# shrubb/latent-pose-reenactment

Measured on AMD Instinct MI355X. Metric: train-step images/sec at 256x256 bs=8, higher is better.
Workload: dtype mixed 16-bit MFMA operands, fp32 accumulate, fp32 activations / weights / optimizer state; 1 GPU; default.yaml meta-training step (configs[2]): ResNeXt50 identity encoder over 8 frames + MobileNetV2 pose encoder (both trained, forward + backward on hand-written gfx950 kernels), G, D with the 98000x512 label embedding, VGG19/VGGFace/featmat/adversarial/dis_embed/dice criterions, Adam, EMA; image_size=256, per_gpu_batch=8, global_batch=8, parallelism=dp1, precision_mode=default assignment (LP_PREC=f16), padding=zero, launch_mode=hipgraph

## Files before the change

### latent_pose_reenactment_amd/build.py

```python
import os
import subprocess
import sys
import time
from concurrent.futures import ThreadPoolExecutor

HERE = os.path.dirname(os.path.abspath(__file__))
CSRC = os.path.join(HERE, 'csrc')
INCLUDE = os.path.join(os.path.dirname(HERE), 'include')
LIB = os.path.join(HERE, 'liblp_hip.so')
SOURCES = ['lp_api.hip', 'elementwise.hip', 'norm_bwd.hip', 'tanh_head.hip', 'spectral_norm.hip', 'act_pack.hip', 'conv_dma.hip', 'conv_pipe.hip', 'conv_wgrad.hip', 'conv_thin.hip', 'conv_stem8.hip', 'linear_crop.hip', 'mobilenet.hip', 'resnext.hip', 'reflect_border.hip', 'stickman.hip']
FLAGS = ['--offload-arch=gfx950', '-O3', '-std=c++17', '-fPIC', '-I', INCLUDE, '-I', CSRC]


def _newer(a, b):
    return not os.path.exists(b) or os.path.getmtime(a) > os.path.getmtime(b)


def build(force: bool = False, verbose: bool = True) -> str:
    hipcc = os.environ.get('HIPCC', '/opt/rocm/bin/hipcc')
    objdir = os.path.join(HERE, 'build')
    os.makedirs(objdir, exist_ok=True)
    headers = [os.path.join(CSRC, f) for f in os.listdir(CSRC) if f.endswith('.h')] + [os.path.join(INCLUDE, 'lp_hip.h')]
    jobs = []
    for src in SOURCES:
        s = os.path.join(CSRC, src)
        o = os.path.join(objdir, src.replace('.hip', '.o'))
        if force or _newer(s, o) or any(_newer(h, o) for h in headers):
            jobs.append((s, o))

    def compile_one(job):
        s, o = job
        t_start = time.time()
        cmd = [hipcc] + FLAGS + ['-c', s, '-o', o]
        if verbose:
            print('[lp build]', ' '.join(cmd), flush=True)
        r = subprocess.run(cmd, capture_output=True, text=True)
        if r.returncode != 0:
            raise RuntimeError(f'hipcc failed for {s}:\n{r.stderr}')
        os.utime(o, (t_start, t_start))
        return o

    with ThreadPoolExecutor(max_workers=4) as ex:
        list(ex.map(compile_one, jobs))
    objs = [os.path.join(objdir, s.replace('.hip', '.o')) for s in SOURCES]
    if jobs or not os.path.exists(LIB):
        cmd = [hipcc, '--offload-arch=gfx950', '-shared', '-fPIC', '-o', LIB] + objs
        if verbose:
            print('[lp build]', ' '.join(cmd), flush=True)
        r = subprocess.run(cmd, capture_output=True, text=True)
        if r.returncode != 0:
            raise RuntimeError(f'link failed:\n{r.stderr}')
    return LIB


if __name__ == '__main__':
    print(build(force='--force' in sys.argv))
```

### latent_pose_reenactment_amd/csrc/conv_common.h

```cpp
#pragma once
#include "lp_common.h"
#include <stdlib.h>

struct Conv16Params {
    const uint16_t* a_hi; const uint16_t* a_lo; const uint16_t* w_hi; const uint16_t* w_lo;
    float* y;
    const float* bias; const float* res; const float* alpha; const float* alpha2;
    const uint16_t* mask16;
    uint16_t* o_hi; uint16_t* o_lo;
    int o_relu;
    float* amax;
    float* part; long long part_bytes;
    int N, H, W, Hin, Win, Cin, C8, Cout, Co8, CinP, CoutP;
    int res_shift;
    int lTH, lTW, lNB, tiles_x, tiles_y;
    int hit;
    int a_dbuf;
    int ksplit;
    float* stats;
    long long stats_cap;
    int stats_rows;
    int xcd_map, ntiles, nco;
    int phase;
    int grouped;
};

static inline int ilog2_floor(int v) { int l = 0; while ((1 << (l + 1)) <= v) ++l; return l; }

__device__ __forceinline__ bool conv16_block(const Conv16Params& p, int& tile, int& cob) {
    if (!p.xcd_map) { tile = (int)blockIdx.x; cob = (int)blockIdx.y; return true; }
    const int id = (int)blockIdx.x, x = id & 7, j = id >> 3;
    if (p.xcd_map == 2) { tile = id % p.ntiles; cob = id / p.ntiles; return cob < p.nco; }
    const int per = (p.ntiles + 7) >> 3;
    cob = j % p.nco;
    const int k = j / p.nco;
    tile = x * per + k;
    return k < per && tile < p.ntiles;
}

static inline dim3 conv16_grid(Conv16Params& p, int ntiles, int nco, int gz = 1) {
    static const int on = getenv("LP_CONV_XCD") ? atoi(getenv("LP_CONV_XCD")) : 1;
    p.ntiles = ntiles; p.nco = nco;
    p.xcd_map = (on && nco > 1 && ntiles >= 16) ? on : 0;
    if (!p.xcd_map) return dim3(ntiles, nco, gz);
    return dim3(((ntiles + 7) / 8) * 8 * nco, 1, gz);
}

static inline void choose_tile(int BM, int N, int H, int W, int* lTH, int* lTW, int* lNB) {
    int lbm = ilog2_floor(BM);
    int ltw = ilog2_floor(W); if (ltw > 4) ltw = 4;
    int lth = ilog2_floor(H); if (lth > lbm - ltw) lth = lbm - ltw;
    if (lth < 1) lth = 1;
    if (ltw < 1) ltw = 1;
    int lnb = lbm - ltw - lth; if (lnb < 0) lnb = 0;
    while (lnb > 0 && (1 << (lnb - 1)) >= N) --lnb;
    *lTH = lth; *lTW = ltw; *lNB = lnb;
}

int lp_conv_pipe_launch(Conv16Params& p, int ups, int prec, hipStream_t s);
int lp_conv1x1_pipe_launch(Conv16Params& p, int prec, hipStream_t s);

template <int WM, int WN, int MR, int NR, int PREC, int MRP>
__device__ __forceinline__ void conv16_epilogue(const Conv16Params& p, f32x4_t (&acc)[MR][NR], unsigned char* smem, int wave_d, int wm, int wn,
                                                int lane, int n0, int y0, int x0, int co0, int NBv, int tile_index, int ph = -1) {
    constexpr bool SPLIT = (PREC == LP_PREC_BF16X3), F16 = (PREC == LP_PREC_F16);
    float alpha = p.alpha ? *p.alpha : 1.f;
    if (p.alpha2) alpha *= *p.alpha2;
    if ((p.Cout & 3) == 0) {
        constexpr int WR = MR * 16, WC = NR * 16, LDW = WC + 4;
        __syncthreads();
        float* tile = (float*)smem + wave_d * (MRP * 16 * LDW);
        constexpr int C4 = WC / 4;
        constexpr int RPP = 64 / C4;
        const int c4 = lane % C4, rsub = lane / C4;
        const int co = co0 + wn * WC + c4 * 4;
        float4 bv = make_float4(0.f, 0.f, 0.f, 0.f);
        if (p.bias && co < p.Cout) bv = *(const float4*)(p.bias + co);
        float am = 0.f;
        float st_n = 0.f, st_ref[4] = {0.f, 0.f, 0.f, 0.f}, st_d[4] = {0.f, 0.f, 0.f, 0.f}, st_q[4] = {0.f, 0.f, 0.f, 0.f};
#pragma unroll
        for (int mp = 0; mp < MR; mp += MRP) {
#pragma unroll
            for (int mr = mp; mr < mp + MRP; ++mr)
#pragma unroll
                for (int nr = 0; nr < NR; ++nr)
#pragma unroll
                    for (int r = 0; r < 4; ++r)
                        tile[((mr - mp) * 16 + (lane >> 4) * 4 + r) * LDW + nr * 16 + (lane & 15)] = acc[mr][nr][r];
#pragma unroll 4
        for (int r0 = mp * 16; r0 < (mp + MRP) * 16; r0 += RPP) {
            const int row = r0 + rsub;
            const int m = wm * WR + row;
            int nb, py, px;
            tile_row_linear(m, p.lTH, p.lTW, nb, py, px);
            const int n = n0 + nb;
            int oyy = y0 + py, oxx = x0 + px;
            bool inside = nb < NBv && n < p.N && co < p.Cout;
            if (ph >= 0) { inside = inside && oyy < p.Hin && oxx < p.Win; oyy = 2 * oyy + (ph >> 1); oxx = 2 * oxx + (ph & 1); }
            else inside = inside && oyy < p.H && oxx < p.W;
            if (inside) {
                float4 v = *(const float4*)(tile + (row - mp * 16) * LDW + c4 * 4);
                if (p.ksplit > 1) {
                    const size_t pixs = (size_t)(n * p.H + oyy) * p.W + oxx;
                    *(float4*)(p.part + ((size_t)blockIdx.z * p.N * p.H * p.W + pixs) * p.Cout + co) = v;
                    continue;
                }
                v.x = fmaf(v.x, alpha, bv.x); v.y = fmaf(v.y, alpha, bv.y); v.z = fmaf(v.z, alpha, bv.z); v.w = fmaf(v.w, alpha, bv.w);
                if (p.res) {
                    const float4 rv = *(const float4*)(p.res + ((size_t)(n * (p.H >> p.res_shift) + (oyy >> p.res_shift)) * (p.W >> p.res_shift)
                                                                + (oxx >> p.res_shift)) * p.Cout + co);
                    v.x += rv.x; v.y += rv.y; v.z += rv.z; v.w += rv.w;
                }
                const size_t pix = (size_t)(n * p.H + oyy) * p.W + oxx;
                if (p.mask16) {
                    const ushort4 mv = *(const ushort4*)(p.mask16 + pix * p.Co8 + co);
                    v.x = (mv.x - 1u) < 0x7fffu ? v.x : 0.f; v.y = (mv.y - 1u) < 0x7fffu ? v.y : 0.f;
                    v.z = (mv.z - 1u) < 0x7fffu ? v.z : 0.f; v.w = (mv.w - 1u) < 0x7fffu ? v.w : 0.f;
                }
                if (p.o_relu & 2) { v.x = fmaxf(v.x, 0.f); v.y = fmaxf(v.y, 0.f); v.z = fmaxf(v.z, 0.f); v.w = fmaxf(v.w, 0.f); }
                if (p.y) *(float4*)(p.y + pix * p.Cout + co) = v;
                am = lp_amax4(am, v);
                if (p.stats) {
                    const float o4[4] = {v.x, v.y, v.z, v.w};
                    if (st_n == 0.f) { st_ref[0] = v.x; st_ref[1] = v.y; st_ref[2] = v.z; st_ref[3] = v.w; }
#pragma unroll
                    for (int j = 0; j < 4; ++j) { const float d = o4[j] - st_ref[j]; st_d[j] += d; st_q[j] = fmaf(d, d, st_q[j]); }
                    st_n += 1.f;
                }
                if (p.o_hi) {
                    float o[4] = {v.x, v.y, v.z, v.w};
                    ushort4 oh, ol;
                    uint16_t* ohp = (uint16_t*)&oh; uint16_t* olp = (uint16_t*)&ol;
#pragma unroll
                    for (int j = 0; j < 4; ++j) {
                        const float q = (p.o_relu & 1) ? fmaxf(o[j], 0.f) : o[j];
                        ohp[j] = lp_f32_to_op16<F16>(q);
                        if (SPLIT) olp[j] = lp_f32_to_op16<false>(q - lp_op16_to_f32<false>(ohp[j]));
                    }
                    *(ushort4*)(p.o_hi + pix * p.Co8 + co) = oh;
                    if (SPLIT) *(ushort4*)(p.o_lo + pix * p.Co8 + co) = ol;
                }
            }
        }
        }
        if (p.amax && p.ksplit == 1) lp_amax_commit(am, p.amax, blockIdx.x + blockIdx.y * 7u);
        if (p.stats && p.ksplit == 1) {
            float mean[4], m2[4];
#pragma unroll
            for (int j = 0; j < 4; ++j) {
                mean[j] = 0.f; m2[j] = 0.f;
                if (st_n > 0.f) { mean[j] = st_ref[j] + st_d[j] / st_n; m2[j] = fmaxf(st_q[j] - st_d[j] * st_d[j] / st_n, 0.f); }
            }
#pragma unroll
            for (int o = C4; o < 64; o <<= 1) {
                const float nb_ = __shfl_xor(st_n, o, 64);
                float mb[4], qb[4];
#pragma unroll
                for (int j = 0; j < 4; ++j) { mb[j] = __shfl_xor(mean[j], o, 64); qb[j] = __shfl_xor(m2[j], o, 64); }
                const float nn = st_n + nb_;
                if (nn > 0.f) {
                    const float fb = nb_ / nn, fab = st_n * fb;
#pragma unroll
                    for (int j = 0; j < 4; ++j) { const float d = mb[j] - mean[j]; mean[j] = fmaf(d, fb, mean[j]); m2[j] += qb[j] + d * d * fab; }
                }
                st_n = nn;
            }
            if (rsub == 0 && co < p.Cout) {
                float* o = p.stats + ((size_t)(tile_index * WM + wm) * p.Cout + co) * 3;
#pragma unroll
                for (int j = 0; j < 4; ++j) { o[j * 3 + 0] = st_n; o[j * 3 + 1] = mean[j]; o[j * 3 + 2] = m2[j]; }
            }
        }
        return;
    }
    float am_s = 0.f;
#pragma unroll
    for (int mr = 0; mr < MR; ++mr) {
#pragma unroll
        for (int r = 0; r < 4; ++r) {
            const int m = wm * (MR * 16) + mr * 16 + (lane >> 4) * 4 + r;
            int nb, py, px;
            tile_row_linear(m, p.lTH, p.lTW, nb, py, px);
            const int n = n0 + nb, oyy = y0 + py, oxx = x0 + px;
            if (nb >= NBv || n >= p.N || oyy >= p.H || oxx >= p.W) continue;
            const size_t pixi = (size_t)(n * p.H + oyy) * p.W + oxx;
            const size_t pix = pixi * p.Cout;
            size_t rpix = 0;
            if (p.res) rpix = ((size_t)(n * (p.H >> p.res_shift) + (oyy >> p.res_shift)) * (p.W >> p.res_shift) + (oxx >> p.res_shift)) * p.Cout;
#pragma unroll
            for (int nr = 0; nr < NR; ++nr) {
                const int co = co0 + wn * (NR * 16) + nr * 16 + (lane & 15);
                if (co < p.Cout) {
                    float v = acc[mr][nr][r] * alpha;
                    if (p.bias) v += p.bias[co];
                    if (p.res) v += p.res[rpix + co];
                    if (p.mask16 && !((unsigned)(p.mask16[pixi * p.Co8 + co] - 1u) < 0x7fffu)) v = 0.f;
                    if (p.y) p.y[pix + co] = v;
                    am_s = fmaxf(am_s, fabsf(v));
                    if (p.o_hi) {
                        const float q = (p.o_relu & 1) ? fmaxf(v, 0.f) : v;
                        const uint16_t h = lp_f32_to_op16<F16>(q);
                        p.o_hi[pixi * p.Co8 + co] = h;
                        if (SPLIT) p.o_lo[pixi * p.Co8 + co] = lp_f32_to_op16<false>(q - lp_op16_to_f32<false>(h));
                    }
                }
            }
        }
    }
    if (p.amax) lp_amax_commit(am_s, p.amax, blockIdx.x + blockIdx.y * 7u);
}
```

### latent_pose_reenactment_amd/csrc/conv_dma.hip

```cpp
#include "lp_common.h"
#include "conv_common.h"
#include "lp_hip.h"
#include "lp_internal.h"
#include <stdlib.h>
#include <type_traits>

__device__ __attribute__((aligned(64))) unsigned int lp_zero_page[16];


template <int KS, bool UPS, int WM, int WN, int MR, int NR, int PREC, bool PP, int NBUF = 2, int CC = 32, bool GH = false>
#ifndef LP_PP_MINW
#define LP_PP_MINW 2
#endif
#ifndef LP_X3_1X1_MINW
#define LP_X3_1X1_MINW 3
#endif
__global__ __launch_bounds__(WM * WN * 64 * (PP ? 2 : 1), (PP && PREC != LP_PREC_BF16X3) ? LP_PP_MINW : (!PP && NBUF == 2 && WM * WN == 4 && PREC != LP_PREC_BF16X3) ? 2 :
                             (KS == 1 && !PP && WM * WN == 4 && PREC == LP_PREC_BF16X3) ? LP_X3_1X1_MINW : 1)
void conv_dma_kernel(Conv16Params p) {
    constexpr int ROWB = CC * 2;
    constexpr int SL = CC / 8, RPI = 64 / SL;
    constexpr int KK = CC / 32;
    static_assert(CC == 32 || CC == 64, "32- or 64-channel chunks");
    constexpr bool SPLIT = (PREC == LP_PREC_BF16X3), F16 = (PREC == LP_PREC_F16);
// ... 276 lines not shown
        float4 v = *(const float4*)(p.part + i * 4);
        for (int z = 1; z < p.ksplit; ++z) {
            const float4 q = *(const float4*)(p.part + z * slice + i * 4);
            v.x += q.x; v.y += q.y; v.z += q.z; v.w += q.w;
        }
        float4 bv = make_float4(0.f, 0.f, 0.f, 0.f);
        if (p.bias) bv = *(const float4*)(p.bias + co);
        v.x = fmaf(v.x, alpha, bv.x); v.y = fmaf(v.y, alpha, bv.y); v.z = fmaf(v.z, alpha, bv.z); v.w = fmaf(v.w, alpha, bv.w);
        if (p.res) {
            const int ox = (int)(pix % p.W); const size_t t = pix / p.W;
            const int oy = (int)(t % p.H), n = (int)(t / p.H);
            const float4 rv = *(const float4*)(p.res + ((size_t)(n * (p.H >> p.res_shift) + (oy >> p.res_shift)) * (p.W >> p.res_shift)
                                                        + (ox >> p.res_shift)) * p.Cout + co);
            v.x += rv.x; v.y += rv.y; v.z += rv.z; v.w += rv.w;
        }
        if (p.mask16) {
            const ushort4 mv = *(const ushort4*)(p.mask16 + pix * p.Co8 + co);
            v.x = (mv.x - 1u) < 0x7fffu ? v.x : 0.f; v.y = (mv.y - 1u) < 0x7fffu ? v.y : 0.f;
            v.z = (mv.z - 1u) < 0x7fffu ? v.z : 0.f; v.w = (mv.w - 1u) < 0x7fffu ? v.w : 0.f;
        }
        if (p.o_relu & 2) { v.x = fmaxf(v.x, 0.f); v.y = fmaxf(v.y, 0.f); v.z = fmaxf(v.z, 0.f); v.w = fmaxf(v.w, 0.f); }
        if (p.y) *(float4*)(p.y + pix * p.Cout + co) = v;
        am = lp_amax4(am, v);
        if (p.o_hi) {
            float o[4] = {v.x, v.y, v.z, v.w};
            ushort4 oh, ol;
            uint16_t* ohp = (uint16_t*)&oh; uint16_t* olp = (uint16_t*)&ol;
#pragma unroll
            for (int j = 0; j < 4; ++j) {
                const float q = (p.o_relu & 1) ? fmaxf(o[j], 0.f) : o[j];
                ohp[j] = lp_f32_to_op16<F16>(q);
                if (SPLIT) olp[j] = lp_f32_to_op16<false>(q - lp_op16_to_f32<false>(ohp[j]));
            }
            *(ushort4*)(p.o_hi + pix * p.Co8 + co) = oh;
            if (SPLIT) *(ushort4*)(p.o_lo + pix * p.Co8 + co) = ol;
        }
    }
    if (p.amax) lp_amax_commit(am, p.amax, blockIdx.x);
}

template <int KS, bool UPS, int WM, int WN, int MR, int NR, int PREC, bool PP, int NBUF = 2, int CC = 32, bool GH = false>
static int launch_v(Conv16Params& p, size_t lds, dim3 grid, hipStream_t stream) {
    auto kern = conv_dma_kernel<KS, UPS, WM, WN, MR, NR, PREC, PP, NBUF, CC, GH>;
    static thread_local int attr_dev = -1;
    int dev = 0;
    if (hipGetDevice(&dev) != hipSuccess) return lp_set_error(LP_ERR_HIP, "hipGetDevice failed");
    if (attr_dev != dev) {
        if (hipFuncSetAttribute((const void*)kern, hipFuncAttributeMaxDynamicSharedMemorySize, 160 * 1024) != hipSuccess)
            return lp_set_error(LP_ERR_HIP, "hipFuncSetAttribute failed");
        attr_dev = dev;
    }
    hipLaunchKernelGGL(kern, grid, dim3(WM * WN * 64 * (PP ? 2 : 1)), lds, stream, p);
    return lp_check_launch("conv_dma");
}

template <int KS, bool UPS, int WM, int WN, int MR, int NR, int PREC, int CC = 32, bool GH = false>
static int launch_conv16(Conv16Params& p, hipStream_t stream) {
    constexpr int BM = WM * MR * 16, BN = WN * NR * 16, NWAVE = WM * WN;
    constexpr bool SPLIT = (PREC == LP_PREC_BF16X3);
    constexpr int ROWB = CC * 2, RPI = 64 / (CC / 8);
    constexpr size_t B_BUF = (size_t)KS * BN * ROWB * (SPLIT ? 2 : 1);
    constexpr size_t LDS_MAX = 160 * 1024;
    constexpr int AIT = ((BM == 128) ? (NWAVE == 8 ? 3 : 5) : 6) * (CC / 32) - (CC == 64 ? 1 : 0);
    if (p.CinP % CC) return lp_set_error(LP_ERR_ARG, "conv16: padded input channels must be a multiple of the chunk size");
    const bool phf = (KS == 2) && p.phase == 1, phd = (KS == 2) && p.phase == 2;
    const int GHt = phf ? p.Hin : p.H, GWt = phf ? p.Win : p.W;
    choose_tile(BM, p.N, GHt, GWt, &p.lTH, &p.lTW, &p.lNB);
    int HH, HW, halo_px;
    for (;;) {
        const int TH = 1 << p.lTH, TW = 1 << p.lTW, NBv = 1 << p.lNB;
        if (KS == 1) { HH = TH; HW = TW; } else if (KS == 2) { HH = TH + 1; HW = TW + 1; } else if (UPS) { HH = TH / 2 + 2; HW = TW / 2 + 2; } else { HH = TH + 2; HW = TW + 2; }
        halo_px = NBv * HH * HW;
        if ((halo_px + RPI - 1) / RPI <= AIT * NWAVE || p.lNB == 0) break;
        --p.lNB;
    }
    const int TH = 1 << p.lTH, TW = 1 << p.lTW, NBv = 1 << p.lNB;
    p.tiles_x = (GWt + TW - 1) / TW; p.tiles_y = (GHt + TH - 1) / TH;
    const int NH = (halo_px + RPI - 1) / RPI;
    p.hit = (NH + NWAVE - 1) / NWAVE;
    if (p.hit > AIT) return lp_set_error(LP_ERR_UNSUPPORTED, "conv16: halo exceeds the DMA descriptor budget");
    const size_t a_buf = (size_t)p.hit * NWAVE * 1024 * (SPLIT ? 2 : 1);
    static const int adbuf_env = getenv("LP_CONV_ADBUF") ? atoi(getenv("LP_CONV_ADBUF")) : -1;
    p.a_dbuf = (2 * a_buf + 2 * B_BUF <= LDS_MAX) ? 1 : 0;
    if (adbuf_env == 0 && KS == 1) p.a_dbuf = 0;
    if (adbuf_env < 0 && KS == 1 && SPLIT && CC == 32 && p.CinP <= 256) p.a_dbuf = 0;
    static const int b1_env = getenv("LP_CONV1X1_B1") ? atoi(getenv("LP_CONV1X1_B1")) : 0;
    const bool b1 = KS == 1 && CC == 32 && ((b1_env && !p.a_dbuf) || (b1_env >= 2 && SPLIT && BN == 128));
    if (b1) p.a_dbuf = 1;
    const size_t lds_halo = (p.a_dbuf ? 2 : 1) * a_buf;
    size_t lds = lds_halo + (b1 ? 1 : 2) * B_BUF;
    size_t epi = (size_t)NWAVE * ((KS == 1) ? 16 : MR * 16) * (NR * 16 + 4) * sizeof(float);
    const int tiles = p.tiles_x * p.tiles_y * ((p.N + NBv - 1) / NBv) * (phf ? 4 : 1);
    constexpr bool pp_ok = (KS == 3 || KS == 2) && (NWAVE == 4);
    static const int pp_env = getenv("LP_CONV_PP") ? atoi(getenv("LP_CONV_PP")) : -1;
    const long long pp_wgs = (long long)((tiles + 1) / 2) * ((p.Cout + BN - 1) / BN);
    const bool pp = pp_ok && (pp_env >= 0 ? pp_env != 0 : pp_wgs >= 200) && tiles >= 2 && p.a_dbuf && (!phf || ((p.tiles_x * p.tiles_y) & 1) == 0);
    if (pp) epi *= 2;
    if (lds < epi) lds = epi;
    if (lds > LDS_MAX) return lp_set_error(LP_ERR_UNSUPPORTED, "conv16 tile needs too much LDS");
    dim3 grid(pp ? (tiles + 1) / 2 : tiles, (p.Cout + BN - 1) / BN);
    p.xcd_map = 0; p.ntiles = grid.x; p.nco = grid.y;
    {
        static const int max_split = getenv("LP_CONV_KSPLIT") ? atoi(getenv("LP_CONV_KSPLIT")) : 8;
        static const int split_wgs = getenv("LP_CONV_SPLIT_WGS") ? atoi(getenv("LP_CONV_SPLIT_WGS")) : 256;
        const int wgs = grid.x * grid.y, nch = (p.CinP / CC) * (phd ? 4 : 1);
        int ks = 1;
        if ((KS == 3 || KS == 2) && (p.Cout & 3) == 0 && p.part)
            while (ks < max_split && wgs * ks * 2 <= split_wgs && nch / (ks * 2) >= 2 &&
                   (long long)(ks * 2) * p.N * p.H * p.W * p.Cout * (long long)sizeof(float) <= p.part_bytes) ks *= 2;
        for (;;) { const int per = (nch + ks - 1) / ks, k2 = (nch + per - 1) / per; if (k2 == ks) break; ks = k2; }
        p.ksplit = ks;
        grid.z = ks;
    }
    if ((KS == 3 || KS == 2) && !p.grouped) grid = conv16_grid(p, (int)grid.x, (int)grid.y, (int)grid.z);
    p.stats_rows = 0;
    if (p.stats) {
        constexpr int WR = MR * 16;
        const long long rows = (long long)(pp ? 2 * ((tiles + 1) / 2) : tiles) * WM;
        const bool ok = (NBv * TH * TW == BM) && (TH * TW >= WR) && (GHt % TH == 0) && (GWt % TW == 0) && ((p.Cout & 3) == 0) && p.ksplit == 1 &&
                        rows * p.Cout * 3 <= p.stats_cap && (!phf || NBv == 1);
        if (ok) p.stats_rows = (p.H * p.W) / WR; else p.stats = nullptr;
    }
    if constexpr (pp_ok) { if (pp) return launch_v<KS, UPS, WM, WN, MR, NR, PREC, true, 2, CC, GH>(p, lds, grid, stream); }
    if constexpr (KS == 1 && CC == 32 && !GH) { if (b1) return launch_v<KS, UPS, WM, WN, MR, NR, PREC, false, 1, CC, GH>(p, lds, grid, stream); }
    constexpr int NQ = KS * BN * ROWB / 1024;
    constexpr bool ring_ok = (NQ % NWAVE == 0);
    static const int nbuf_env = getenv("LP_CONV_NBUF") ? atoi(getenv("LP_CONV_NBUF")) : 0;
    if constexpr (ring_ok) {
        const size_t lds3 = lds_halo + 3 * B_BUF;
        const long long total_wgs = (long long)grid.x * grid.y * grid.z;
        const bool ring = (nbuf_env ? nbuf_env == 3 : total_wgs <= 320) && lds3 <= LDS_MAX;
        if (ring) return launch_v<KS, UPS, WM, WN, MR, NR, PREC, false, 3, CC, GH>(p, lds3 > epi ? lds3 : epi, grid, stream);
    }
    return launch_v<KS, UPS, WM, WN, MR, NR, PREC, false, 2, CC, GH>(p, lds, grid, stream);
}

template <int PREC>
static int dispatch_conv16(Conv16Params& p, int ks, int ups, hipStream_t s) {
    if (ks == 3 && ups >= 2) {
        const int gh = ups == 2 ? p.Hin : p.H, gw = ups == 2 ? p.Win : p.W;
        if ((p.Cout & 3) || gh < 2 || gw < 2) return lp_set_error(LP_ERR_UNSUPPORTED, "phase-decomposed conv: Cout % 4 == 0, low-resolution grid >= 2 x 2");
        if (p.Cout <= 64 && gh * gw >= 256) return launch_conv16<2, false, 4, 1, 4, 4, PREC>(p, s);
        return launch_conv16<2, false, 2, 2, 4, 4, PREC>(p, s);
    }
    if (ks == 3) {
        const int r = lp_conv_pipe_launch(p, ups, PREC, s);
        if (r) return r < 0 ? r : LP_OK;
    }
    if (ks == 1 && !ups) {
        const int r = lp_conv1x1_pipe_launch(p, PREC, s);
        if (r) return r < 0 ? r : LP_OK;
    }
    const bool big_img = p.H * p.W >= 256;
    static const int w8_env = getenv("LP_CONV_W8") ? atoi(getenv("LP_CONV_W8")) : -1;
    const bool w8 = w8_env >= 0 ? (w8_env != 0) : (p.H * p.W <= 256);
    if (w8 && p.Cout > 64) {
        static const int x3bn64 = getenv("LP_CONV_X3_BN64") ? atoi(getenv("LP_CONV_X3_BN64")) : 1;
        if (PREC == LP_PREC_BF16X3 && x3bn64 && ks == 3) {
            if (!ups) return launch_conv16<3, false, 2, 2, 4, 2, PREC>(p, s);
            return launch_conv16<3, true, 2, 2, 4, 2, PREC>(p, s);
        }
        if (ks == 3 && !ups) return launch_conv16<3, false, 2, 4, 4, 2, PREC>(p, s);
        if (ks == 3 && ups) return launch_conv16<3, true, 2, 4, 4, 2, PREC>(p, s);
        if (ks == 1 && !ups) return launch_conv16<1, false, 2, 4, 4, 2, PREC>(p, s);
    }
    if (PREC == LP_PREC_BF16X3 && ks == 3 && p.Cout > 64) {
        static const int x3mid = getenv("LP_CONV_X3_BN64") ? atoi(getenv("LP_CONV_X3_BN64")) : 1;
        const long long tiles128 = ((long long)p.N * p.H * p.W + 127) / 128;
        if (x3mid >= 2 && ((tiles128 + 1) / 2) * ((p.Cout + 127) / 128) < 200) {
            if (!ups) return launch_conv16<3, false, 2, 2, 4, 2, PREC>(p, s);
            return launch_conv16<3, true, 2, 2, 4, 2, PREC>(p, s);
        }
    }
    if (ks == 3 && !ups) {
        if (p.Cout <= 16 && big_img) return launch_conv16<3, false, 4, 1, 4, 1, PREC>(p, s);
        if (p.Cout <= 64 && big_img) return launch_conv16<3, false, 4, 1, 4, 4, PREC>(p, s);
        return launch_conv16<3, false, 2, 2, 4, 4, PREC>(p, s);
    }
    if (ks == 3 && ups) {
        if (p.Cout <= 64 && big_img) return launch_conv16<3, true, 4, 1, 4, 4, PREC>(p, s);
        return launch_conv16<3, true, 2, 2, 4, 4, PREC>(p, s);
    }
    if (ks == 1 && !ups) {
        static const int cc_env = getenv("LP_CONV_CC1") ? atoi(getenv("LP_CONV_CC1")) : 0;
        const bool cc64 = (cc_env ? cc_env == 64 : (p.Cin >= 512 && PREC != LP_PREC_BF16X3)) && (p.CinP % 64 == 0);
        static const int tile_env = getenv("LP_CONV1X1_TILE") ? atoi(getenv("LP_CONV1X1_TILE")) : 0;
        const long long pix = (long long)p.N * p.H * p.W;
        const bool tall = (tile_env ? tile_env == 256 : false) && p.Cout >= 128 && p.H * p.W >= 256 &&
                          (pix / 256) * ((p.Cout + 127) / 128) >= 512;
        if (cc64) {
            if (p.Cout <= 64 && big_img) return launch_conv16<1, false, 4, 1, 4, 4, PREC, 64>(p, s);
            if (tall) return launch_conv16<1, false, 4, 2, 4, 4, PREC, 64>(p, s);
            return launch_conv16<1, false, 2, 2, 4, 4, PREC, 64>(p, s);
        }
        if (p.Cout <= 64 && big_img) return launch_conv16<1, false, 4, 1, 4, 4, PREC>(p, s);
        if (tall) return launch_conv16<1, false, 4, 2, 4, 4, PREC>(p, s);
        return launch_conv16<1, false, 2, 2, 4, 4, PREC>(p, s);
    }
    return lp_set_error(LP_ERR_UNSUPPORTED, "unsupported conv configuration");
}

extern "C" long long lp_conv16_fwd_workspace_bytes(int N, int H, int W, int Cout, int ksize) {
    if (ksize != 3 || (Cout & 3)) return 0;
    const long long P = (long long)N * H * W;
    const long long wgs_lb = ((P + 255) / 256) * ((Cout + 127) / 128);
    static const int max_split = getenv("LP_CONV_KSPLIT") ? atoi(getenv("LP_CONV_KSPLIT")) : 8;
    static const int split_wgs = getenv("LP_CONV_SPLIT_WGS") ? atoi(getenv("LP_CONV_SPLIT_WGS")) : 256;
    long long ks = split_wgs / wgs_lb; if (ks > max_split) ks = max_split;
    if (ks < 2) return 0;
    return ks * P * Cout * (long long)sizeof(float);
}

extern "C" int lp_conv16_fwd(const uint16_t* a_hi, const uint16_t* a_lo, const uint16_t* w_hi, const uint16_t* w_lo, float* y,
                             const float* bias, const float* res, const float* alpha, const float* alpha2,
                             int N, int H, int W, int Cin, int Cout, int CinP, int CoutP,
                             int ksize, int upsample, int res_shift, int prec, const uint16_t* relu_mask16,
                             uint16_t* out_hi, uint16_t* out_lo, int out_relu, float* workspace, long long workspace_bytes, float* amax_slots,
                             void* stream) {
    if (!y) return lp_set_error(LP_ERR_ARG, "lp_conv16_fwd: null pointer");
    return lp_conv16_fwd_stats(a_hi, a_lo, w_hi, w_lo, y, bias, res, alpha, alpha2, N, H, W, Cin, Cout, CinP, CoutP, ksize, upsample, res_shift, prec,
                               relu_mask16, out_hi, out_lo, out_relu, workspace, workspace_bytes, amax_slots, nullptr, 0, nullptr, stream);
}

extern "C" int lp_conv16_fwd_stats(const uint16_t* a_hi, const uint16_t* a_lo, const uint16_t* w_hi, const uint16_t* w_lo, float* y,
                                   const float* bias, const float* res, const float* alpha, const float* alpha2,
                                   int N, int H, int W, int Cin, int Cout, int CinP, int CoutP,
                                   int ksize, int upsample, int res_shift, int prec, const uint16_t* relu_mask16,
                                   uint16_t* out_hi, uint16_t* out_lo, int out_relu, float* workspace, long long workspace_bytes, float* amax_slots,
                                   float* stats, long long stats_capacity_floats, int* stats_rows, void* stream) {
    if (stats_rows) *stats_rows = 0;
    if (!a_hi || !w_hi) return lp_set_error(LP_ERR_ARG, "lp_conv16_fwd: null pointer");
    if (!y && (!out_hi || (Cout & 7))) return lp_set_error(LP_ERR_ARG, "lp_conv16_fwd: y may only be NULL when out_hi is given and Cout % 8 == 0");
    if (stats && !stats_rows) return lp_set_error(LP_ERR_ARG, "lp_conv16_fwd: stats needs stats_rows");
    if (prec == LP_PREC_BF16X3 && (!w_lo || !a_lo)) return lp_set_error(LP_ERR_ARG, "lp_conv16_fwd: bf16x3 needs the lo planes");
    if (prec == LP_PREC_BF16X3 && out_hi && !out_lo) return lp_set_error(LP_ERR_ARG, "lp_conv16_fwd: bf16x3 needs out_lo");
    if ((upsample == 1 || upsample == 2) && ((H | W) & 1)) return lp_set_error(LP_ERR_ARG, "lp_conv16_fwd: upsampled output dims must be even");
    if (upsample < 0 || upsample > 3) return lp_set_error(LP_ERR_ARG, "lp_conv16_fwd: upsample = 0 | 1 | 2 (phase form) | 3 (phase form of the data gradient)");
    if (CinP % 32 || CinP < Cin || CoutP % 128 || CoutP < Cout) return lp_set_error(LP_ERR_ARG, "lp_conv16_fwd: bad padded dims");
    if (H < 2 || W < 2) return lp_set_error(LP_ERR_UNSUPPORTED, "lp_conv16_fwd: H,W must be >= 2");
    Conv16Params p;
    p.a_hi = a_hi; p.a_lo = a_lo; p.w_hi = w_hi; p.w_lo = w_lo; p.y = y; p.bias = bias; p.res = res; p.alpha = alpha; p.alpha2 = alpha2;
    p.mask16 = relu_mask16; p.o_relu = out_relu; p.part = workspace; p.part_bytes = workspace ? workspace_bytes : 0; p.amax = amax_slots;
    p.o_hi = (Cout & 7) ? nullptr : out_hi; p.o_lo = (Cout & 7) ? nullptr : out_lo;
    p.N = N; p.H = H; p.W = W; p.Hin = upsample ? H / 2 : H; p.Win = upsample ? W / 2 : W;
    p.Cin = Cin; p.C8 = (Cin + 7) & ~7; p.Cout = Cout; p.Co8 = (Cout + 7) & ~7; p.CinP = CinP; p.CoutP = CoutP; p.res_shift = res_shift;
    p.grouped = 0; p.stats = stats; p.stats_cap = stats ? stats_capacity_floats : 0; p.stats_rows = 0;
    p.phase = (upsample == 2) ? 1 : (upsample == 3) ? 2 : 0;
    if (upsample >= 2 && ksize != 3) return lp_set_error(LP_ERR_ARG, "lp_conv16_fwd: upsample = 2 | 3 (phase-decomposed forms) are 3x3 forms");
    if (upsample == 3) { p.Hin = 2 * H; p.Win = 2 * W; }
    hipStream_t s = (hipStream_t)stream;
    int rc;
    if (prec == LP_PREC_BF16) rc = dispatch_conv16<LP_PREC_BF16>(p, ksize, upsample, s);
    else if (prec == LP_PREC_BF16X3) rc = dispatch_conv16<LP_PREC_BF16X3>(p, ksize, upsample, s);
    else if (prec == LP_PREC_F16) rc = dispatch_conv16<LP_PREC_F16>(p, ksize, upsample, s);
    else return lp_set_error(LP_ERR_ARG, "lp_conv16_fwd: unknown precision mode");
    if (rc) return rc;
    if (p.ksplit > 1) {
        const long long items = (long long)N * H * W * (Cout >> 2);
        long long blocks = (items + 255) / 256; if (blocks > 2048) blocks = 2048;
        if (prec == LP_PREC_BF16) hipLaunchKernelGGL(splitk_reduce_kernel<LP_PREC_BF16>, dim3((unsigned)blocks), dim3(256), 0, s, p);
        else if (prec == LP_PREC_BF16X3) hipLaunchKernelGGL(splitk_reduce_kernel<LP_PREC_BF16X3>, dim3((unsigned)blocks), dim3(256), 0, s, p);
        else hipLaunchKernelGGL(splitk_reduce_kernel<LP_PREC_F16>, dim3((unsigned)blocks), dim3(256), 0, s, p);
        rc = lp_check_launch("splitk_reduce");
        if (rc) return rc;
    }
    if (stats_rows) *stats_rows = p.stats_rows;
    if (out_hi && !p.o_hi)
        return lp_act_pack(y, nullptr, nullptr, (out_relu & 1) ? 2 : 0, out_hi, out_lo, N, H * W, Cout, prec, nullptr, nullptr, 0, 1, nullptr, stream);
    return LP_OK;
}

extern "C" int lp_gconv16_fwd(const uint16_t* a_hi, const uint16_t* a_lo, const uint16_t* w_hi, const uint16_t* w_lo, float* y,
                              const float* alpha2, int N, int H, int W, int C, int CP, int prec, float* amax_slots, void* stream) {
    return lp_gconv16_fwd_stats(a_hi, a_lo, w_hi, w_lo, y, alpha2, N, H, W, C, CP, prec, amax_slots, nullptr, 0, nullptr, stream);
}

extern "C" int lp_gconv16_fwd_stats(const uint16_t* a_hi, const uint16_t* a_lo, const uint16_t* w_hi, const uint16_t* w_lo, float* y,
                                    const float* alpha2, int N, int H, int W, int C, int CP, int prec, float* amax_slots,
                                    float* stats, long long stats_capacity_floats, int* stats_rows, void* stream) {
    if (!y) return lp_set_error(LP_ERR_ARG, "lp_gconv16_fwd: null pointer");
    return lp_gconv16_fwd_planes(a_hi, a_lo, w_hi, w_lo, y, nullptr, nullptr, alpha2, N, H, W, C, CP, 0, prec, amax_slots, stats,
                                 stats_capacity_floats, stats_rows, stream);
}

extern "C" int lp_gconv16_fwd_planes(const uint16_t* a_hi, const uint16_t* a_lo, const uint16_t* w_hi, const uint16_t* w_lo, float* y,
                                     uint16_t* o_hi, uint16_t* o_lo, const float* alpha2, int N, int H, int W, int C, int CP, int group_size,
                                     int prec, float* amax_slots, float* stats, long long stats_capacity_floats, int* stats_rows,
                                     void* stream) {
    if (stats_rows) *stats_rows = 0;
    if (stats && !stats_rows) return lp_set_error(LP_ERR_ARG, "lp_gconv16_fwd: stats needs stats_rows");
    if (!a_hi || !w_hi || (!y && !o_hi)) return lp_set_error(LP_ERR_ARG, "lp_gconv16_fwd: null pointer");
    if (o_hi && prec == LP_PREC_BF16X3 && !o_lo) return lp_set_error(LP_ERR_ARG, "lp_gconv16_fwd: bf16x3 output planes need lo");
    if (prec == LP_PREC_BF16X3 && (!w_lo || !a_lo)) return lp_set_error(LP_ERR_ARG, "lp_gconv16_fwd: bf16x3 needs the lo planes");
    if ((C & 63) || CP % 128 || CP < C) return lp_set_error(LP_ERR_UNSUPPORTED, "lp_gconv16_fwd: C must be a multiple of 64, CP of 128");
    if (H < 2 || W < 2) return lp_set_error(LP_ERR_UNSUPPORTED, "lp_gconv16_fwd: H,W must be >= 2");
    Conv16Params p;
    p.a_hi = a_hi; p.a_lo = a_lo; p.w_hi = w_hi; p.w_lo = w_lo; p.y = y; p.bias = nullptr; p.res = nullptr; p.alpha = nullptr; p.alpha2 = alpha2;
    p.mask16 = nullptr; p.o_relu = 0; p.part = nullptr; p.part_bytes = 0; p.amax = amax_slots; p.o_hi = o_hi; p.o_lo = o_lo;
    p.N = N; p.H = H; p.W = W; p.Hin = H; p.Win = W;
    p.Cin = C; p.C8 = C; p.Cout = C; p.Co8 = C; p.CinP = 64; p.CoutP = CP; p.res_shift = 0; p.grouped = 1; p.phase = 0;
    p.stats = stats; p.stats_cap = stats ? stats_capacity_floats : 0; p.stats_rows = 0;
    hipStream_t s = (hipStream_t)stream;
    int rc;
    static const bool half_env = !(getenv("LP_GCONV_HALF") && atoi(getenv("LP_GCONV_HALF")) == 0);
    const bool gh = half_env && group_size >= 1 && group_size <= 32 && (32 % group_size) == 0;
    if (prec == LP_PREC_BF16) rc = gh ? launch_conv16<3, false, 4, 1, 4, 4, LP_PREC_BF16, 32, true>(p, s) : launch_conv16<3, false, 4, 1, 4, 4, LP_PREC_BF16>(p, s);
    else if (prec == LP_PREC_BF16X3) rc = gh ? launch_conv16<3, false, 4, 1, 4, 4, LP_PREC_BF16X3, 32, true>(p, s) : launch_conv16<3, false, 4, 1, 4, 4, LP_PREC_BF16X3>(p, s);
    else if (prec == LP_PREC_F16) rc = gh ? launch_conv16<3, false, 4, 1, 4, 4, LP_PREC_F16, 32, true>(p, s) : launch_conv16<3, false, 4, 1, 4, 4, LP_PREC_F16>(p, s);
    else return lp_set_error(LP_ERR_ARG, "lp_gconv16_fwd: unknown precision mode");
    if (stats_rows) *stats_rows = p.stats_rows;
    return rc;
}

extern "C" long long lp_conv16_stats_floats(int N, int H, int W, int Cout) {
    return ((long long)N * H * W / 64 + 16) * Cout * 3;
}
```

Before: 198.7 images/s.

## Add persistent row-tiled grouped-conv kernel with weights held in registers

Adds a dedicated persistent kernel for grouped 3x3 convolutions with group sizes 4/8/16. Each workgroup keeps one 64-channel block of weights in registers, loops over 4x16 spatial tiles, and double-buffers halo loads into swizzled LDS via global-to-LDS DMA. It emits outputs, packed 16-bit planes, amax and per-patch stats in the same pass. The aim is to cut the wasted MFMA work and weight reloading of the generic dense-tile path used for ResNeXt grouped convs. In exchange it adds a large new code path that falls back when shapes are not tile-exact.

```diff
diff --git a/latent_pose_reenactment_amd/build.py b/latent_pose_reenactment_amd/build.py
--- a/latent_pose_reenactment_amd/build.py
+++ b/latent_pose_reenactment_amd/build.py
@@ -8,7 +8,7 @@
 CSRC = os.path.join(HERE, 'csrc')
 INCLUDE = os.path.join(os.path.dirname(HERE), 'include')
 LIB = os.path.join(HERE, 'liblp_hip.so')
-SOURCES = ['lp_api.hip', 'elementwise.hip', 'norm_bwd.hip', 'tanh_head.hip', 'spectral_norm.hip', 'act_pack.hip', 'conv_dma.hip', 'conv_pipe.hip', 'conv_wgrad.hip', 'conv_thin.hip', 'conv_stem8.hip', 'linear_crop.hip', 'mobilenet.hip', 'resnext.hip', 'reflect_border.hip', 'stickman.hip']
+SOURCES = ['lp_api.hip', 'elementwise.hip', 'norm_bwd.hip', 'tanh_head.hip', 'spectral_norm.hip', 'act_pack.hip', 'conv_dma.hip', 'conv_pipe.hip', 'gconv_rows.hip', 'conv_wgrad.hip', 'conv_thin.hip', 'conv_stem8.hip', 'linear_crop.hip', 'mobilenet.hip', 'resnext.hip', 'reflect_border.hip', 'stickman.hip']
 FLAGS = ['--offload-arch=gfx950', '-O3', '-std=c++17', '-fPIC', '-I', INCLUDE, '-I', CSRC]
 
 
diff --git a/latent_pose_reenactment_amd/csrc/conv_common.h b/latent_pose_reenactment_amd/csrc/conv_common.h
--- a/latent_pose_reenactment_amd/csrc/conv_common.h
+++ b/latent_pose_reenactment_amd/csrc/conv_common.h
@@ -59,6 +59,7 @@
 
 int lp_conv_pipe_launch(Conv16Params& p, int ups, int prec, hipStream_t s);
 int lp_conv1x1_pipe_launch(Conv16Params& p, int prec, hipStream_t s);
+int lp_gconv_rows_launch(Conv16Params& p, int group_size, int prec, hipStream_t s);
 
 template <int WM, int WN, int MR, int NR, int PREC, int MRP>
 __device__ __forceinline__ void conv16_epilogue(const Conv16Params& p, f32x4_t (&acc)[MR][NR], unsigned char* smem, int wave_d, int wm, int wn,
diff --git a/latent_pose_reenactment_amd/csrc/conv_dma.hip b/latent_pose_reenactment_amd/csrc/conv_dma.hip
--- a/latent_pose_reenactment_amd/csrc/conv_dma.hip
+++ b/latent_pose_reenactment_amd/csrc/conv_dma.hip
@@ -602,6 +602,11 @@
     p.stats = stats; p.stats_cap = stats ? stats_capacity_floats : 0; p.stats_rows = 0;
     hipStream_t s = (hipStream_t)stream;
     int rc;
+    rc = lp_gconv_rows_launch(p, group_size, prec, s);
+    if (rc) {
+        if (rc > 0 && stats_rows) *stats_rows = p.stats_rows;
+        return rc > 0 ? LP_OK : rc;
+    }
     static const bool half_env = !(getenv("LP_GCONV_HALF") && atoi(getenv("LP_GCONV_HALF")) == 0);
     const bool gh = half_env && group_size >= 1 && group_size <= 32 && (32 % group_size) == 0;
     if (prec == LP_PREC_BF16) rc = gh ? launch_conv16<3, false, 4, 1, 4, 4, LP_PREC_BF16, 32, true>(p, s) : launch_conv16<3, false, 4, 1, 4, 4, LP_PREC_BF16>(p, s);
diff --git a/latent_pose_reenactment_amd/csrc/gconv_rows.hip b/latent_pose_reenactment_amd/csrc/gconv_rows.hip
--- /dev/null
+++ b/latent_pose_reenactment_amd/csrc/gconv_rows.hip
@@ -0,0 +1,257 @@
+#include "lp_common.h"
+#include "conv_common.h"
+#include "lp_hip.h"
+#include "lp_internal.h"
+#include <stdlib.h>
+
+#if defined(__HIP_DEVICE_COMPILE__)
+#pragma clang attribute push(__attribute__((target("no-packed-fp32-ops"))), apply_to = function)
+#endif
+
+static __device__ __attribute__((aligned(64))) unsigned int gr_zero_page[16];
+
+static __device__ __forceinline__ void gr_barrier() {
+    __builtin_amdgcn_fence(__ATOMIC_RELEASE, "workgroup");
+    __builtin_amdgcn_s_barrier();
+    __builtin_amdgcn_fence(__ATOMIC_ACQUIRE, "workgroup");
+}
+static __device__ __forceinline__ float gr_shfl_xor(float v, int lane, int o) {
+    return __builtin_bit_cast(float, __builtin_amdgcn_ds_bpermute((lane ^ o) << 2, __builtin_bit_cast(int, v)));
+}
+
+struct GconvRowsParams {
+    const uint16_t* a_hi; const uint16_t* a_lo; const uint16_t* w_hi; const uint16_t* w_lo;
+    float* y; uint16_t* o_hi; uint16_t* o_lo; const float* alpha2; float* amax; float* stats;
+    int N, H, W, C, CP;
+    int tiles_x, tiles_y, ntiles;
+    int nblk, wgs, xcd;
+};
+
+namespace gr {
+constexpr int TH = 4, TW = 16, HH = TH + 2, HW = TW + 2, HALO_PX = HH * HW;
+constexpr int PIECES = (HALO_PX * 128 + 1023) / 1024;
+constexpr int PLANE = PIECES * 1024;
+constexpr int KIT = (PIECES + 3) / 4;
+__host__ __device__ constexpr int key(int hp) { return ((hp >> 1) & 3) << 1; }
+}
+
+template <int PREC>
+__global__ __launch_bounds__(256, PREC == LP_PREC_BF16X3 ? 2 : 4) void gconv_rows_kernel(GconvRowsParams p) {
+    using namespace gr;
+    constexpr bool SPLIT = (PREC == LP_PREC_BF16X3), F16 = (PREC == LP_PREC_F16);
+    constexpr int BUF = PLANE * (SPLIT ? 2 : 1);
+    extern __shared__ __attribute__((aligned(16))) unsigned char smem[];
+
+    const int lane = (int)threadIdx.x & 63;
+    const int wave = __builtin_amdgcn_readfirstlane((int)threadIdx.x >> 6);
+    const int kb = lane >> 4, px = lane & 15;
+
+    int blk, t0, tstep, tend;
+    {
+        const int id = (int)blockIdx.x;
+        if (p.xcd) {
+            const int x = id & 7, j = id >> 3, per = (p.ntiles + 7) >> 3;
+            blk = j % p.nblk;
+            tstep = p.wgs >> 3;
+            t0 = x * per + j / p.nblk;
+            tend = min(x * per + per, p.ntiles);
+        } else {
+            blk = id % p.nblk;
+            tstep = p.wgs;
+            t0 = id / p.nblk;
+            tend = p.ntiles;
+        }
+    }
+    if (t0 >= tend) return;
+    const int co0 = blk * 64;
+
+    s16x8_t whi[5], wlo[5];
+#pragma unroll
+    for (int s = 0; s < 5; ++s) {
+        const int tap = 2 * s + (lane >> 5);
+        whi[s] = (s16x8_t){0, 0, 0, 0, 0, 0, 0, 0};
+        wlo[s] = (s16x8_t){0, 0, 0, 0, 0, 0, 0, 0};
+        if (tap < 9) {
+            const size_t off = ((size_t)tap * p.CP + co0 + 16 * wave + px) * 64 + 16 * wave + 8 * (kb & 1);
+            whi[s] = *(const s16x8_t*)(p.w_hi + off);
+            if (SPLIT) wlo[s] = *(const s16x8_t*)(p.w_lo + off);
+        }
+    }
+    const float alpha = p.alpha2 ? *p.alpha2 : 1.f;
+
+    int r_off[TH][5];
+#pragma unroll
+    for (int s = 0; s < 5; ++s) {
+        const int tap = min(2 * s + (lane >> 5), 8);
+#pragma unroll
+        for (int r = 0; r < TH; ++r) {
+            const int hp = (r + tap / 3) * HW + px + tap % 3;
+            r_off[r][s] = hp * 128 + (((2 * wave + (kb & 1)) ^ key(hp)) << 4);
+        }
+    }
+
+    int d_hy[KIT], d_hx[KIT], d_c[KIT];
+#pragma unroll
+    for (int k = 0; k < KIT; ++k) {
+        const int hp = (4 * k + wave) * 8 + (lane >> 3);
+        d_hy[k] = hp < HALO_PX ? hp / HW : -(1 << 20);
+        d_hx[k] = hp % HW;
+        d_c[k] = co0 + (((lane & 7) ^ key(hp)) << 3);
+    }
+    const uint16_t* zero16 = (const uint16_t*)gr_zero_page;
+    const unsigned lds0 = (unsigned)__builtin_amdgcn_readfirstlane((int)(unsigned)(uintptr_t)smem);
+    auto decode = [&](int t, int& n, int& y0, int& x0) {
+        x0 = (t % p.tiles_x) * TW; t /= p.tiles_x;
+        y0 = (t % p.tiles_y) * TH; n = t / p.tiles_y;
+    };
+    auto issue = [&](int t, int buf) {
+        int n, y0, x0;
+        decode(t, n, y0, x0);
+#pragma unroll
+        for (int k = 0; k < KIT; ++k) {
+            const int q = 4 * k + wave;
+            if (q < PIECES) {
+                const int iy = y0 - 1 + d_hy[k], ix = x0 - 1 + d_hx[k];
+                const bool ok = iy >= 0 && iy < p.H && ix >= 0 && ix < p.W;
+                const size_t off = ok ? ((size_t)(n * p.H + iy) * p.W + ix) * p.C + d_c[k] : 0;
+                const unsigned d = lds0 + (unsigned)(buf * BUF + q * 1024);
+                lp_glds16(ok ? (p.a_hi + off) : zero16, d);
+                if (SPLIT) lp_glds16(ok ? (p.a_lo + off) : zero16, d + PLANE);
+            }
+        }
+    };
+
+    float am = 0.f;
+    issue(t0, 0);
+    int buf = 0;
+    for (int t = t0; t < tend; t += tstep, buf ^= 1) {
+        lp_wait_vm0();
+        gr_barrier();
+        if (t + tstep < tend) issue(t + tstep, buf ^ 1);
+        int n, y0, x0;
+        decode(t, n, y0, x0);
+        const unsigned char* Hb = smem + buf * BUF;
+        float st_ref[4] = {0.f, 0.f, 0.f, 0.f}, st_d[4] = {0.f, 0.f, 0.f, 0.f}, st_q[4] = {0.f, 0.f, 0.f, 0.f};
+#pragma unroll
+        for (int r = 0; r < TH; ++r) {
+            f32x4_t acc = (f32x4_t){0.f, 0.f, 0.f, 0.f};
+            int lhalf = lane >> 5;
+            asm volatile("" : "+v"(lhalf));
+#pragma unroll
+            for (int s = 0; s < 5; ++s) {
+                const s16x8_t bh = *(const s16x8_t*)(Hb + r_off[r][s]);
+                s16x8_t bl;
+                if (SPLIT) bl = *(const s16x8_t*)(Hb + PLANE + r_off[r][s]);
+#pragma unroll
+                for (int h = 0; h < 2; ++h) {
+                    if (2 * s + h > 8) continue;
+                    const s16x8_t zero = (s16x8_t){0, 0, 0, 0, 0, 0, 0, 0};
+                    const s16x8_t mh = (lhalf == h) ? whi[s] : zero;
+                    if (SPLIT) {
+                        const s16x8_t ml = (lhalf == h) ? wlo[s] : zero;
+                        acc = mfma16t<false>(mh, bl, acc);
+                        acc = mfma16t<false>(ml, bh, acc);
+                    }
+                    acc = mfma16t<F16>(mh, bh, acc);
+                }
+            }
+            const int oy = y0 + r, ox = x0 + px;
+            float4 v;
+            v.x = fmaf(acc[0], alpha, 0.f); v.y = fmaf(acc[1], alpha, 0.f); v.z = fmaf(acc[2], alpha, 0.f); v.w = fmaf(acc[3], alpha, 0.f);
+            if (p.stats) {
+                const float o4[4] = {v.x, v.y, v.z, v.w};
+#pragma unroll
+                for (int k = 0; k < 4; ++k)
+#pragma unroll
+                    for (int j = 0; j < 4; ++j) {
+                        const float xv = __builtin_bit_cast(float, __builtin_amdgcn_ds_bpermute(((lane & 48) | (4 * k + (px & 3))) << 2, __builtin_bit_cast(int, o4[j])));
+                        if (r == 0 && k == 0) st_ref[j] = xv;
+                        const float d = xv - st_ref[j];
+                        st_d[j] += d; st_q[j] = fmaf(d, d, st_q[j]);
+                    }
+            }
+            if (oy < p.H && ox < p.W) {
+                const size_t e = (((size_t)n * p.H + oy) * p.W + ox) * p.C + co0 + 16 * wave + 4 * kb;
+                if (p.y) *(float4*)(p.y + e) = v;
+                am = lp_amax4(am, v);
+                if (p.o_hi) {
+                    const float o[4] = {v.x, v.y, v.z, v.w};
+                    ushort4 oh, ol;
+                    uint16_t* ohp = (uint16_t*)&oh; uint16_t* olp = (uint16_t*)&ol;
+#pragma unroll
+                    for (int j = 0; j < 4; ++j) {
+                        ohp[j] = lp_f32_to_op16<F16>(o[j]);
+                        if (SPLIT) olp[j] = lp_f32_to_op16<false>(o[j] - lp_op16_to_f32<false>(ohp[j]));
+                    }
+                    *(ushort4*)(p.o_hi + e) = oh;
+                    if (SPLIT) *(ushort4*)(p.o_lo + e) = ol;
+                }
+            }
+        }
+        if (p.stats) {
+            float cnt = 16.f, mean[4], m2[4];
+#pragma unroll
+            for (int j = 0; j < 4; ++j) { mean[j] = st_ref[j] + st_d[j] / cnt; m2[j] = fmaxf(st_q[j] - st_d[j] * st_d[j] / cnt, 0.f); }
+#pragma unroll
+            for (int o = 1; o < 4; o <<= 1) {
+#pragma unroll
+                for (int j = 0; j < 4; ++j) {
+                    const float mb = gr_shfl_xor(mean[j], lane, o), qb = gr_shfl_xor(m2[j], lane, o);
+                    const float d = mb - mean[j];
+                    mean[j] = fmaf(d, 0.5f, mean[j]); m2[j] += qb + d * d * (cnt * 0.5f);
+                }
+                cnt *= 2.f;
+            }
+            if (px == 0) {
+                const int ty = y0 >> 2;
+                const int rb = ((n * (p.tiles_y >> 2) + (ty >> 2)) * p.tiles_x + (x0 >> 4)) * 4 + (ty & 3);
+                float* o = p.stats + ((size_t)rb * p.C + co0 + 16 * wave + 4 * kb) * 3;
+#pragma unroll
+                for (int j = 0; j < 4; ++j) { o[j * 3 + 0] = cnt; o[j * 3 + 1] = mean[j]; o[j * 3 + 2] = m2[j]; }
+            }
+        }
+    }
+    if (p.amax) lp_amax_commit(am, p.amax, blockIdx.x);
+}
+
+#if defined(__HIP_DEVICE_COMPILE__)
+#pragma clang attribute pop
+#endif
+
+int lp_gconv_rows_launch(Conv16Params& c, int group_size, int prec, hipStream_t s) {
+    static const int mode = getenv("LP_GCONV_ROWS") ? atoi(getenv("LP_GCONV_ROWS")) : 1;
+    static const int wgs_cap = getenv("LP_GCONV_ROWS_WGS") ? atoi(getenv("LP_GCONV_ROWS_WGS")) : 0;
+    if (mode == 0 || !(group_size == 4 || group_size == 8 || group_size == 16)) return 0;
+    if (prec != LP_PREC_BF16 && prec != LP_PREC_BF16X3 && prec != LP_PREC_F16) return 0;
+    const bool exact = (c.W % gr::TW == 0) && (c.H % gr::TH == 0);
+    if (mode != 2 && !exact) return 0;
+    const bool patches = (c.W % 16 == 0) && (c.H % 16 == 0);
+    if (c.stats && !patches && (c.H * c.W) % 64 == 0) return 0;
+    GconvRowsParams p;
+    p.a_hi = c.a_hi; p.a_lo = c.a_lo; p.w_hi = c.w_hi; p.w_lo = c.w_lo; p.y = c.y; p.o_hi = c.o_hi; p.o_lo = c.o_lo; p.alpha2 = c.alpha2; p.amax = c.amax;
+    p.N = c.N; p.H = c.H; p.W = c.W; p.C = c.Cout; p.CP = c.CoutP;
+    p.tiles_x = (c.W + gr::TW - 1) / gr::TW; p.tiles_y = (c.H + gr::TH - 1) / gr::TH; p.ntiles = c.N * p.tiles_x * p.tiles_y;
+    p.nblk = c.Cout / 64;
+    c.stats_rows = 0;
+    if (c.stats) {
+        const long long rows = (long long)c.N * (c.H * c.W / 64);
+        if (patches && rows * c.Cout * 3 <= c.stats_cap) c.stats_rows = c.H * c.W / 64; else c.stats = nullptr;
+    }
+    p.stats = c.stats;
+    const int occ = prec == LP_PREC_BF16X3 ? 2 : 4;
+    static int cus = 0;
+    if (!cus) { int dev = 0; if (hipGetDevice(&dev) != hipSuccess || hipDeviceGetAttribute(&cus, hipDeviceAttributeMultiprocessorCount, dev) != hipSuccess || cus < 1) cus = 256; }
+    int wgs = (cus * occ + p.nblk - 1) / p.nblk;
+    if (wgs_cap > 0 && wgs > wgs_cap) wgs = wgs_cap;
+    if (wgs > p.ntiles) wgs = p.ntiles;
+    p.xcd = (wgs >= 8 && p.ntiles >= 16) ? 1 : 0;
+    if (p.xcd) wgs &= ~7;
+    p.wgs = wgs;
+    const dim3 grid((unsigned)(p.nblk * wgs));
+    const size_t lds = 2 * gr::PLANE * (prec == LP_PREC_BF16X3 ? 2 : 1);
+    if (prec == LP_PREC_BF16X3) hipLaunchKernelGGL(gconv_rows_kernel<LP_PREC_BF16X3>, grid, dim3(256), lds, s, p);
+    else if (prec == LP_PREC_F16) hipLaunchKernelGGL(gconv_rows_kernel<LP_PREC_F16>, grid, dim3(256), lds, s, p);
+    else hipLaunchKernelGGL(gconv_rows_kernel<LP_PREC_BF16>, grid, dim3(256), lds, s, p);
+    const int rc = lp_check_launch("gconv_rows");
+    return rc ? rc : 1;
+}
```

After: 202.7 images/s (median of 6 runs). 1.02x the previous value.
